# demox-labs/aleo

Hardware: AMD Instinct MI355X
Metric: MSM G1 scalar-muls/sec (2^20 bases per GPU, BLS12-377, bit-exact) (higher is better)
Workload: dtype u32

## Files before the change

aleo_amd/csrc/bases.hip:

```cpp
#include "entry.h"
#include "g2.h"
#include <cstdlib>
#include <cstring>

namespace aleo_mi355x {

struct RowFormat { size_t packed, strided; int32_t (*unpack)(Ctx* c, const void* d_rows, void* d_xy, void* d_flags, size_t n, hipStream_t s); };
static int32_t unpack_g2_200(Ctx* c, const void* d_rows, void* d_xy, void* d_flags, size_t n, hipStream_t s) {
  return g2_unpack200(d_rows, d_xy, d_flags, (uint32_t*)((char*)d_flags + ((n + 3) & ~(size_t)3)), n, s);
}
static constexpr RowFormat G1_ROWS = {96, 104, unpack_affine104}, G2_ROWS = {192, 200, unpack_g2_200};

static int32_t stage_rows(Ctx* c, const RowFormat& f, const void* rows, size_t stride, size_t n, void* d_xy, void* d_raw, void* d_flags, uint32_t* n_inf) {
  *n_inf = 0;
  if (!n) return ALEO_MI355X_OK;
  if (stride == f.packed) { HIPCHK(hipMemcpyAsync(d_xy, rows, n * f.packed, hipMemcpyHostToDevice, c->stream)); return ALEO_MI355X_OK; }
  HIPCHK(hipMemcpyAsync(d_raw, rows, n * f.strided, hipMemcpyHostToDevice, c->stream));
  if (int32_t rc = f.unpack(c, d_raw, d_xy, d_flags, n, c->stream)) return rc;
  HIPCHK(hipMemcpyAsync(n_inf, (char*)d_flags + ((n + 3) & ~(size_t)3), 4, hipMemcpyDeviceToHost, c->stream));
  HIPCHK(hipStreamSynchronize(c->stream));
  return ALEO_MI355X_OK;
}
static int32_t stage_rows_owned(Ctx* c, const RowFormat& f, const void* rows, size_t stride, size_t n, void** d_xy, uint8_t** d_inf) {
  DevTmp raw, flags; uint32_t n_inf = 0; int32_t rc;
// ... 19 lines not shown
}
static int32_t cold_bases(Ctx* c, const void* bases, size_t stride, size_t n, PinnedBases* pb) {
  *pb = PinnedBases(); pb->n = n; int32_t rc; const uint8_t* d_inf = nullptr;
  if ((rc = stage_rows_cold(c, G1_ROWS, bases, stride, n, &d_inf)) || (rc = c->cold_xy28.reserve((n ? n : 1) * ROW28))) return rc;
  pb->d_xy = c->cold_xy.p; pb->d_inf = (uint8_t*)d_inf;
  if ((rc = rows_to28_into(pb->d_xy, c->cold_xy28.p, n, c->stream))) return rc;
  pb->d_xy28 = c->cold_xy28.p;
  return ALEO_MI355X_OK;
}
template <class T> static uint64_t register_set(Device* d, std::map<uint64_t, std::shared_ptr<T>>& table, std::shared_ptr<T> o) {
  std::lock_guard<std::mutex> lk(d->mu);
  uint64_t h = d->next_handle++; table[h] = std::move(o); return h;
}
int32_t find_bases(Device* d, uint64_t handle, std::shared_ptr<PinnedOwner>* keep, PinnedBases* snap) {
  std::lock_guard<std::mutex> lk(d->mu);
  if (int32_t rc = handle_get(d->bases, handle, "unknown bases handle", keep)) return rc;
  *snap = (*keep)->pb; return ALEO_MI355X_OK;
}
template <class T> static int32_t unpin(Device* d, std::map<uint64_t, std::shared_ptr<T>>& table, uint64_t handle, const char* unknown) {
  std::shared_ptr<T> dead;
  std::lock_guard<std::mutex> lk(d->mu);
  return handle_get(table, handle, unknown, &dead, true);
}
static int32_t precompute_once(Ctx* c, const std::shared_ptr<PinnedOwner>& o) {
  Device* d = c->dev; PinnedBases work;
  {
    std::lock_guard<std::mutex> lk(d->mu);
    if (o->pb.tabled || o->building) return ALEO_MI355X_OK;
    o->building = true; work = o->pb;
  }
  int32_t rc = msm_precompute(c, &work);
  std::lock_guard<std::mutex> lk(d->mu);
  o->building = false;
  if (rc == ALEO_MI355X_OK) { for (int i = 0; i < 3; ++i) o->pb.tab[i] = work.tab[i]; o->pb.tabled = true; }
  return rc;
}

static bool looks_sparse(const void* scalars, size_t n) {
  if (n < 4096) return false;
  const uint64_t* s = (const uint64_t*)scalars; size_t small = 0; const size_t step = n / 257;
  for (size_t i = 0; i < 257; ++i) { const uint64_t* v = s + 4 * (i * step); small += (v[1] | v[2] | v[3]) == 0 && v[0] < (1ull << 32); }
  return small >= 129;
}
int32_t msm_host_scalars(Ctx* c, void* out, const PinnedBases& pb, const void* scalars, size_t n, bool mont) {
  const bool skewed = !mont && looks_sparse(scalars, n);
  const bool sparse = skewed && pb.range.d && pb.range_off == 0 && n <= pb.range.cover;
  if (!n) return msm_run1(c, (uint64_t*)out, pb, nullptr, 0, mont, c->stream, false);
  return msm_run1_split(c, (uint64_t*)out, pb, nullptr, n, mont, c->stream, sparse, scalars, !skewed);
}

static uint64_t hash96(const uint8_t* p) {
  uint64_t h = 1469598103934665603ull;
  for (int i = 0; i < 96; ++i) { h ^= p[i]; h *= 1099511628211ull; }
  return h;
}
static constexpr size_t SRS_SAMPLES = 256, SRS_CACHE_ENTRIES = 8, SRS_MIN_N = 1024;

static bool srs_cache_enabled() {
  const char* e = std::getenv("ALEO_MI355X_SRS_CACHE");
  return e && e[0] == '1';
}
static SrsCacheEntry* srs_lookup(Device* d, const void* bases, size_t stride, size_t n) {
  for (auto& e : d->srs_cache) {
    if (e.host_ptr != bases || e.stride != stride || e.n < n) continue;
    bool ok = true; size_t checked = 0;
    for (auto& sm : e.samples) {
      if (sm.first >= n) continue;
// ... 94 lines not shown
  });
}

int32_t aleo_mi355x_bases_generate(const void* base104, uint64_t first, size_t n, uint64_t* handle) {
  return guarded([&] {
    if (!base104 || !handle) return ALEO_MI355X_ERR_BAD_ARG;
    return pin_new(handle, [&](Ctx* c, std::shared_ptr<PinnedOwner>* o) { *o = std::make_shared<PinnedOwner>(); return generate_multiples(c, base104, first, n, &(*o)->pb); });
  });
}

int32_t aleo_mi355x_bases_from_scalars(const void* base104, const void* scalars, size_t n, uint64_t* handle) {
  return guarded([&] {
    if (!base104 || !handle || !scalars) return ALEO_MI355X_ERR_BAD_ARG;
    return pin_new(handle, [&](Ctx* c, std::shared_ptr<PinnedOwner>* o) { *o = std::make_shared<PinnedOwner>(); return generate_from_scalars(c, base104, scalars, n, &(*o)->pb); });
  });
}

int32_t aleo_mi355x_bases_precompute(uint64_t handle) {
  return guarded([&] {
    Slot sl; if (sl.rc) return sl.rc;
    FoundBases fb(sl.d, handle); if (fb.rc) return fb.rc;
    return precompute_once(sl.c, fb.keep);
  });
}

int32_t aleo_mi355x_bases_precompute_range(uint64_t handle, size_t offset, size_t n, int32_t window_bits) {
  return guarded([&] {
    Slot sl; if (sl.rc) return sl.rc;
    std::shared_ptr<PinnedOwner> keep; PinnedBases work; { int32_t rcb = find_bases(sl.d, handle, &keep, &work); if (rcb) return rcb; }
    { std::lock_guard<std::mutex> g(sl.d->mu); if (keep->building) return bad_arg("bases_precompute_range: a table build is in flight"); keep->building = true; work = keep->pb; }
    int32_t rc = msm_precompute_range(sl.c, &work, offset, n, window_bits);
    std::lock_guard<std::mutex> g(sl.d->mu);
    keep->building = false;
    if (rc == ALEO_MI355X_OK) { keep->pb.range = work.range; keep->pb.range_off = work.range_off; }
    return rc;
  });
}

int32_t aleo_mi355x_bases_info(uint64_t handle, uint64_t* out, int32_t cap) {
  return guarded([&] {
    if (!out || cap <= 0) return 0;
    Device* d = nullptr; if (get_device(&d)) return 0;
    std::shared_ptr<PinnedOwner> keep; PinnedBases pb; if (find_bases(d, handle, &keep, &pb)) return 0;
    uint64_t v[8] = {pb.n, pb.n * (96 + ROW28) + (pb.d_inf ? pb.n : 0), 0, 0, 0, 0, 0, 0};
    int k = 0;
    for (const auto& t : pb.tab) if (t.d) { const uint64_t W = (254 + t.c - 1) / t.c; v[2] += W * t.cover * ROW28; v[3 + k] = (uint64_t)t.c; ++k; }
    v[6] = (uint64_t)k;
    const int32_t m = cap < 8 ? cap : 8;
    for (int32_t i = 0; i < m; ++i) out[i] = v[i];
    return m;
  }, 0);
}

int32_t aleo_mi355x_bases_download(uint64_t handle, size_t offset, size_t n, void* out104) {
  return guarded([&] {
    if (!out104 && n) return ALEO_MI355X_ERR_BAD_ARG;
    Slot sl; if (sl.rc) return sl.rc;
    FoundBases fb(sl.d, handle); if (fb.rc) return fb.rc;
    if (offset + n > fb.pb.n) return bad_arg("bases_download: range");
    std::vector<uint8_t> xy(n * 96 + 1), inf(n + 1, 0);
    HIPCHK(hipMemcpy(xy.data(), (const char*)fb.pb.d_xy + offset * 96, n * 96, hipMemcpyDeviceToHost));
    if (fb.pb.d_inf) HIPCHK(hipMemcpy(inf.data(), fb.pb.d_inf + offset, n, hipMemcpyDeviceToHost));
    uint8_t* o = (uint8_t*)out104;
    for (size_t i = 0; i < n; ++i) { std::memcpy(o + i * 104, &xy[i * 96], 96); std::memset(o + i * 104 + 96, 0, 8); o[i * 104 + 96] = inf[i]; }
    return ALEO_MI355X_OK;
  });
}

int32_t aleo_mi355x_bases_unpin(uint64_t handle) {
  return guarded([&] { Slot sl; if (sl.rc) return sl.rc; return unpin(sl.d, sl.d->bases, handle, "unknown bases handle"); });
}

int32_t aleo_mi355x_bases_g2_pin(const void* bases, size_t base_stride, size_t n, uint64_t* handle) {
  return guarded([&] {
    if (!handle || (!bases && n) || (base_stride != 200 && base_stride != 192) || n >= (1ull << 31)) return bad_arg("bases_g2_pin: bad argument");
    Slot sl; if (sl.rc) return sl.rc;
    std::shared_ptr<PinnedG2> o;
    const int32_t rc = g2_upload(sl.c, bases, base_stride, n, &o);
    if (rc) return rc;
// ... 10 lines not shown
```

aleo_amd/csrc/ctx.h:

```cpp
#pragma once
#include <hip/hip_runtime.h>
#include <atomic>
#include <condition_variable>
#include <cstdint>
#include <cstdio>
#include <map>
#include <memory>
#include <functional>
#include <mutex>
#include <string>
#include <vector>
#include "../../include/aleo_mi355x.h"

namespace aleo_mi355x {

extern thread_local std::string g_last_error;

#define HIPCHK(expr)                                                                                   \
  do {                                                                                                 \
    hipError_t e__ = (expr);                                                                           \
    if (e__ != hipSuccess) {                                                                           \
      char buf__[512];                                                                                 \
      snprintf(buf__, sizeof buf__, "%s failed: %s (%s:%d)", #expr, hipGetErrorString(e__), __FILE__, __LINE__); \
      g_last_error = buf__;                                                                            \
      return (e__ == hipErrorOutOfMemory) ? ALEO_MI355X_ERR_OOM : ALEO_MI355X_ERR_HIP;                 \
    }                                                                                                  \
  } while (0)

struct DevBuf {
  void* p = nullptr; size_t cap = 0;
  int32_t reserve(size_t bytes) {
    if (bytes <= cap) return ALEO_MI355X_OK;
    if (p) { (void)hipFree(p); p = nullptr; cap = 0; }
    size_t want = bytes + bytes / 8;
    HIPCHK(hipMalloc(&p, want));
    cap = want; return ALEO_MI355X_OK;
  }
  template <class T> T* as() const { return (T*)p; }
};

struct Carve { size_t total = 0; size_t part(size_t bytes) { const size_t at = total; total += (bytes + 31) & ~(size_t)31; return at; } };

struct DevTmp {
  void* p = nullptr;
  DevTmp() = default; DevTmp(const DevTmp&) = delete; DevTmp& operator=(const DevTmp&) = delete;
  ~DevTmp() { if (p) (void)hipFree(p); }
  int32_t alloc(size_t bytes) { HIPCHK(hipMalloc(&p, bytes ? bytes : 1)); return ALEO_MI355X_OK; }
  void* release() { void* q = p; p = nullptr; return q; }
};

#ifndef ALEO_ROW28
#define ALEO_ROW28 128
#endif
static constexpr size_t ROW28 = ALEO_ROW28;
static_assert(ROW28 == 112 || ROW28 == 128, "row stride of the 28-bit tables");

struct PinnedBases {
  void* d_xy = nullptr;
  void* d_xy28 = nullptr;
  uint8_t* d_inf = nullptr;
  struct PreTable { void* d = nullptr; int c = 0; size_t cover = 0, min_n = 0; };
  PreTable tab[3];
  PreTable range; size_t range_off = 0;
  bool tabled = false;
  uint64_t shards = 0; size_t shard_min = 0;
  size_t shard_ntt_min = (size_t)1 << 24;
  size_t n = 0;
};

struct PinnedOwner {
  PinnedBases pb; bool building = false;
  ~PinnedOwner() { if (pb.d_xy) (void)hipFree(pb.d_xy); if (pb.d_xy28) (void)hipFree(pb.d_xy28); if (pb.d_inf) (void)hipFree(pb.d_inf); for (auto& t : pb.tab) if (t.d) (void)hipFree(t.d); if (pb.range.d) (void)hipFree(pb.range.d); }
};

struct PinnedG2 {
  void* d_xy = nullptr; uint8_t* d_inf = nullptr; void* d_rows28 = nullptr; size_t n = 0;
  ~PinnedG2() { if (d_xy) (void)hipFree(d_xy); if (d_inf) (void)hipFree(d_inf); if (d_rows28) (void)hipFree(d_rows28); }
};

struct SrsCacheEntry {
  const void* host_ptr = nullptr; size_t n = 0, stride = 0; uint64_t handle = 0, last_use = 0; uint32_t hits = 0;
  std::vector<std::pair<size_t, uint64_t>> samples;
};

struct MsmTiming { double total = 0, sort = 0, accum = 0, reduce = 0, host = 0, accum_kernel = 0; int accum_launches = 1; };

struct NttTables;

struct Device;

struct Ctx {
  Device* dev = nullptr;
  int device = -1;
  hipStream_t stream = nullptr;
  std::mutex mu;
  hipEvent_t ev[8] = {};
  uint32_t meta_seq = 0;
// ... 115 lines not shown
```

aleo_amd/csrc/g1_setup.hip:

```cpp
#include "ec.h"
#include "fp28.h"
#include "msm_common.h"

namespace aleo_mi355x {

static constexpr uint32_t GEN_K = 64;
__device__ __constant__ uint32_t FQ_P_MINUS_2[12] = {0xffffffffu, 0x8508bfffu, 0x30000000u, 0x170b5d44u, 0xba094800u, 0x1ef3622fu,
                                                     0x00f5138fu, 0x1a22d9f3u, 0x6ca1493bu, 0xc63b05c0u, 0x17c510eau, 0x01ae3a46u};
__device__ __noinline__ void fq_mul_ni(Fq* r, const Fq* a, const Fq* b) { *r = Fq::mul(*a, *b); }
__device__ __noinline__ void fq_inverse_ni(Fq* io) {
  Fq a = *io, acc = Fq::one();
  for (int bit = 376; bit >= 0; --bit) {
    fq_mul_ni(&acc, &acc, &acc);
    if ((FQ_P_MINUS_2[bit >> 5] >> (bit & 31)) & 1u) fq_mul_ni(&acc, &acc, &a);
  }
  *io = acc;
}

__global__ void __launch_bounds__(256) k_gen_xyzz(const char* __restrict__ g_affine, uint64_t first, uint32_t n, char* __restrict__ tmp) {
  uint32_t t = blockIdx.x * 256 + threadIdx.x;
  uint64_t i0 = (uint64_t)t * GEN_K; if (i0 >= n) return;
  AffinePt g = load_affine(g_affine);
  XYZZ G; G.X = g.x; G.Y = g.y; G.ZZ = Fq::one(); G.ZZZ = Fq::one();
  uint64_t k = first + i0;
  XYZZ acc = xyzz_infinity();
  for (int bit = 63 - __clzll(k); bit >= 0; --bit) {
    xyzz_double_ni(&acc);
    if ((k >> bit) & 1ull) xyzz_add_ni(&acc, &G);
  }
  for (uint32_t j = 0; j < GEN_K && i0 + j < n; ++j) {
    store_xyzz(tmp + (i0 + j) * 192, acc);
    xyzz_add_ni(&acc, &G);
  }
}
// ... 113 lines not shown
  (void)c;
  uint32_t* count = (uint32_t*)((char*)d_flags + ((n + 3) & ~(size_t)3));
  HIPCHK(hipMemsetAsync(count, 0, 4, s));
  const size_t want = (n + 255) / 256;
  hipLaunchKernelGGL(k_unpack104, dim3((uint32_t)(want < 16384 ? want : 16384)), dim3(256), 0, s, (const char*)d_rows104, (char*)d_xy96, (uint8_t*)d_flags, count, n);
  HIPCHK(hipGetLastError());
  return ALEO_MI355X_OK;
}

__global__ void __launch_bounds__(256) k_rows_to28(const char* __restrict__ src96, char* __restrict__ dst112, uint32_t n) {
  uint32_t i = blockIdx.x * 256 + threadIdx.x; if (i >= n) return;
  AffinePt p = load_affine(src96 + (size_t)i * 96);
  F28 x, y;
  if (p.x.is_zero_raw() && p.y.is_zero_raw()) { x = f28_const(Limbs14{}); y = x; }
  else { x = f28_from_fq(p.x); y = f28_from_fq(p.y); }
  store_affine28(dst112 + (size_t)i * ROW28, x, y);
}
int32_t rows_to28_into(const void* d_xy96, void* d_dst, size_t n, hipStream_t s) {
  if (n == 0) return ALEO_MI355X_OK;
  hipLaunchKernelGGL(k_rows_to28, dim3((uint32_t)((n + 255) / 256)), dim3(256), 0, s, (const char*)d_xy96, (char*)d_dst, (uint32_t)n);
  HIPCHK(hipGetLastError());
  return ALEO_MI355X_OK;
}
int32_t make_rows28(Ctx* c, PinnedBases* pb) {
  if (pb->d_xy28 || pb->n == 0) return ALEO_MI355X_OK;
  DevTmp rows; int32_t rc;
  if ((rc = rows.alloc(pb->n * ROW28))) return rc;
  if ((rc = rows_to28_into(pb->d_xy, rows.p, pb->n, c->stream))) return rc;
  HIPCHK(hipStreamSynchronize(c->stream));
  pb->d_xy28 = rows.release();
  return ALEO_MI355X_OK;
}

static int32_t build_table(Ctx* c, const PinnedBases* pb, int pre_c, size_t n, PinnedBases::PreTable* out, size_t off = 0) {
  const uint32_t W = (SCALAR_BITS + pre_c - 1) / pre_c;
  if (n * (size_t)W >= (1ull << 31)) { g_last_error = "bases_precompute: table index would exceed 31 bits"; return ALEO_MI355X_ERR_BAD_ARG; }
  DevTmp tab, cur, prefix, row; int32_t rc;
  if ((rc = tab.alloc(n * ROW28 * W))) return rc;
  if ((rc = cur.alloc(n * 192)) || (rc = prefix.alloc(n * 48)) || (rc = row.alloc(n * 96))) return rc;
  hipStream_t s = c->stream;
  const uint32_t g = (uint32_t)((n + 255) / 256), lanes = (uint32_t)((n + GEN_K - 1) / GEN_K), gl = (lanes + 255) / 256;
  const char* xy = (const char*)pb->d_xy + off * 96;
  if (pb->d_xy28) HIPCHK(hipMemcpyAsync(tab.p, (const char*)pb->d_xy28 + off * ROW28, n * ROW28, hipMemcpyDeviceToDevice, s));
  else hipLaunchKernelGGL(k_rows_to28, dim3(g), dim3(256), 0, s, xy, (char*)tab.p, (uint32_t)n);
  hipLaunchKernelGGL(k_pre_init, dim3(g), dim3(256), 0, s, xy, (uint32_t)n, (char*)cur.p);
  for (uint32_t w = 1; w < W; ++w) {
    hipLaunchKernelGGL(k_pre_double, dim3(g), dim3(256), 0, s, (char*)cur.p, (uint32_t)n, win_width(pre_c, (int)w - 1));
    hipLaunchKernelGGL(k_gen_normalize, dim3(gl), dim3(256), 0, s, (char*)cur.p, (uint32_t)n, (char*)prefix.p, (char*)row.p);
    hipLaunchKernelGGL(k_rows_to28, dim3(g), dim3(256), 0, s, (const char*)row.p, (char*)tab.p + (size_t)w * n * ROW28, (uint32_t)n);
  }
  HIPCHK(hipGetLastError());
  HIPCHK(hipStreamSynchronize(s));
  out->d = tab.release(); out->c = pre_c; out->cover = n;
  return ALEO_MI355X_OK;
}

int32_t msm_precompute(Ctx* c, PinnedBases* pb) {
  if (pb->tabled || pb->n == 0) return ALEO_MI355X_OK;
  const size_t N = pb->n; int32_t rc = ALEO_MI355X_OK; int k = 0;
  auto lim = [&](size_t cap) { return N < cap ? N : cap; };
  auto tier = [&](int cbits, size_t cover, size_t min_n) {
    if (rc) return;
    if ((rc = build_table(c, pb, cbits, cover, &pb->tab[k])) == ALEO_MI355X_OK) pb->tab[k++].min_n = min_n;
  };
  constexpr size_t TIER_SLACK = 64;
  const size_t cover16 = lim(((size_t)1 << 17) + TIER_SLACK), cover13 = lim(((size_t)1 << 15) + TIER_SLACK);
  if (N > cover16) tier(N >= (1u << 19) ? 20 : 17, N, cover16 + 1);
  if (N >= (1u << 15)) tier(16, cover16, (size_t)1 << 15);
  if (N >= (1u << 10)) tier(13, cover13, (size_t)1 << 10);
  if (rc) {
    for (auto& t : pb->tab) { if (t.d) (void)hipFree(t.d); t = PinnedBases::PreTable(); }
    return rc;
  }
  pb->tabled = true;
  return ALEO_MI355X_OK;
}

int32_t msm_precompute_range(Ctx* c, PinnedBases* pb, size_t off, size_t n, int window_bits) {
  if (pb->range.d) { g_last_error = "bases_precompute_range: this set already has a range table"; return ALEO_MI355X_ERR_BAD_ARG; }
  if (!n || off + n > pb->n || (window_bits != 13 && window_bits != 16)) { g_last_error = "bases_precompute_range: bad range or window (13 or 16 bits)"; return ALEO_MI355X_ERR_BAD_ARG; }
  int32_t rc = build_table(c, pb, window_bits, n, &pb->range, off);
  if (rc) return rc;
  pb->range.min_n = 0; pb->range_off = off;
  return ALEO_MI355X_OK;
}

}
```

aleo_amd/csrc/msm.hip:

```cpp
#include "msm_reduce.h"

namespace aleo_mi355x {

__device__ __forceinline__ XYZZ xyzz28_to_xyzz(const XYZZ28& a) {
  XYZZ r; r.X = f28_to_fq(a.X); r.Y = f28_to_fq(a.Y); r.ZZ = f28_to_fq(a.ZZ); r.ZZZ = f28_to_fq(a.ZZZ); return r;
}
__device__ __noinline__ void slice_slow_path28(const char* bases, const uint32_t* run, uint32_t j, uint32_t j1, const XYZZ28* acc28, XYZZ* acc_out, bool* inf_out) {
  XYZZ acc = xyzz28_to_xyzz(*acc28); bool inf = false;
  for (; j < j1; ++j) {
    uint32_t e = run[j];
    F28 x, y; load_affine28(bases + (size_t)(e & 0x7fffffffu) * ROW28, x, y);
    AffinePt p; p.x = Fq::reduce(f28_to_fq(x)); p.y = Fq::reduce(f28_to_fq(y));
    if (e >> 31) p.y = fq_neg_canonical(p.y);
    xyzz_madd(acc, inf, p.x, p.y);
  }
  *acc_out = acc; *inf_out = inf;
}

__device__ __forceinline__ const char* chain_sum(const FrontChain& ch, uint32_t g) {
  for (uint32_t i = 0; i < ch.n; ++i) if (ch.v[i].hist[g]) return ch.v[i].partial + (size_t)scan_at(ch.v[i].scan_local, ch.v[i].scan_blk, g).y * 224u;
  return nullptr;
}

template <bool OUT28, bool SEED = false>
__global__ void __launch_bounds__(256) k_accum28(const char* __restrict__ bases, const uint32_t* __restrict__ sorted, const uint32_t* __restrict__ hist,
                                                 const uint2* __restrict__ scan_local, const uint2* __restrict__ scan_blk, const uint32_t* __restrict__ total_pairs, uint32_t M,
                                                 const uint32_t* __restrict__ meta, const uint32_t* __restrict__ order, const uint32_t* __restrict__ task_g,
                                                 char* __restrict__ partial, FrontChain seed) {
  uint32_t t = blockIdx.x * 256 + threadIdx.x;
  if (t >= meta[0]) return;
  const uint32_t sid = order[t], g = task_g[sid];
  uint2 st = scan_at(scan_local, scan_blk, g);
  uint32_t cnt = hist[g], m = slices_of(cnt, pick_rule(total_pairs, M)), k = sid - st.y;
  uint32_t j0 = (uint32_t)(((uint64_t)k * cnt) / m), j1 = (uint32_t)(((uint64_t)(k + 1) * cnt) / m);
  const uint32_t* run = sorted + st.x;
  uint32_t e_next = run[j0];
  F28 xn, yn; load_affine28(bases + (size_t)(e_next & 0x7fffffffu) * ROW28, xn, yn);
  XYZZ28 acc; bool ok = true;
  uint32_t j = j0;
  bool seeded = false;
  if constexpr (SEED) {
    const char* sp = k == 0 ? chain_sum(seed, g) : nullptr;
    if (sp) {
      acc.ZZ = load_f28(sp + 112);
      if (!f28_is_zero_raw(acc.ZZ)) { acc.X = load_f28(sp); acc.Y = f28_mul(load_f28(sp + 56), f28_const(ONE28)); acc.ZZZ = load_f28(sp + 168); seeded = true; }
    }
  }
  if (!seeded) {
    uint32_t e = e_next; F28 x = xn, y = yn;
    if (j + 1 < j1) { e_next = run[j + 1]; load_affine28(bases + (size_t)(e_next & 0x7fffffffu) * ROW28, xn, yn); }
    if (e >> 31) y = f28_sub<2, 1>(f28_const(Limbs14{}), y);
    acc.X = x; acc.Y = y; acc.ZZ = f28_const(ONE28); acc.ZZZ = f28_const(ONE28);
    ++j;
  }
// ... 240 lines not shown
  ((uint4*)out)[t] = ((const uint4*)(V + (size_t)w * stride * PB28))[q];
}

int32_t msm_front_sort(Ctx* c, const PinnedBases& pb, const MsmJob& job, hipStream_t s, Front& f) {
  const uint32_t K = f.K = job.k;
  size_t n = 0, pts = 0; SegArgs segs{};
  if (K > MAX_SETS || job.nseg > MAX_SEGS) { g_last_error = "msm: too many sets / segments in one call"; return ALEO_MI355X_ERR_BAD_ARG; }
  for (uint32_t q = 0; q < job.nseg; ++q) {
    const MsmSeg& g = job.segs[q];
    if (g.len == 0) continue;
    if (g.out >= K || g.off + g.len >= (1ull << 31)) { g_last_error = "msm: segment out of range"; return ALEO_MI355X_ERR_BAD_ARG; }
    const uint32_t i = segs.nseg++;
    segs.ptr[i] = (const char*)g.d_ptr; segs.n[i] = (uint32_t)g.len; segs.off[i] = (uint32_t)g.off; segs.set[i] = (uint8_t)g.out;
    n = g.off + g.len > n ? g.off + g.len : n; pts += g.len;
  }
  if (n == 0) { f.empty = true; return ALEO_MI355X_OK; }
  if (job.tier_n > n && job.tier_n <= pb.n) n = job.tier_n;
  if (n > pb.n) { g_last_error = "msm: a segment reaches past the pinned bases"; return ALEO_MI355X_ERR_BAD_ARG; }
  const PinnedBases::PreTable* T = nullptr;
  const uint8_t* d_inf = pb.d_inf;
  bool ranged = job.sparse && pb.range.d != nullptr;
  for (uint32_t i = 0; ranged && i < segs.nseg; ++i) ranged = segs.off[i] >= pb.range_off && (size_t)segs.off[i] + segs.n[i] <= pb.range_off + pb.range.cover;
  if (ranged) {
    T = &pb.range; n = 0;
    for (uint32_t i = 0; i < segs.nseg; ++i) { segs.off[i] -= (uint32_t)pb.range_off; n = (size_t)segs.off[i] + segs.n[i] > n ? (size_t)segs.off[i] + segs.n[i] : n; }
    if (d_inf) d_inf += pb.range_off;
  } else T = msm_tier(pb, n);
  const bool pre = f.pre = T != nullptr;
  if (K > 1 && (!pre || K > (ranged ? msm_range_sets(pb) : msm_max_sets(pb, n)))) { g_last_error = "msm: internal: batch without a table tier (or too many sets)"; return ALEO_MI355X_ERR_BAD_ARG; }
  MsmPlan& P = f.P; P = make_plan(pre ? n : pts, pre ? T->c : 0);
  if (pre) { P.W = K; P.M = K * P.B; }
  if (!pre && !pb.d_xy28) { g_last_error = "msm: pinned set without 28-bit rows"; return ALEO_MI355X_ERR_HIP; }
  f.bases = (const char*)(pre ? T->d : pb.d_xy28);
  f.plain_tree = k_tree_pass<Pt32, 2>;
  const uint32_t cpw = f.cpw = P.B / P.S, nchunks = f.nchunks = cpw * P.W;
  uint32_t lgN = 0; while ((1u << lgN) < cpw) ++lgN;
  f.lgN = lgN;
  const bool masked = f.masked = pre && lgN >= 2 && (1u << lgN) == cpw;
  if (pre && !masked) { g_last_error = "msm: internal: table path without masked reduction"; return ALEO_MI355X_ERR_HIP; }
  int32_t rc;
  const uint32_t tseg = f.tseg = cpw / 4, fseg = f.fseg = lgN + 4, nseg = f.nseg = K * fseg, setw = f.setw = fseg * tseg;
  constexpr uint32_t SUM_TREE_MIN_C = 13;
  f.prog = masked && P.c >= SUM_TREE_MIN_C && cpw > FOLD;
  f.out_pts = f.prog ? 1 + lgN : fseg;
  f.vpoints = masked ? (size_t)K * setw + nchunks + (nseg + 1) + (size_t)nseg * (tseg / 2 + tseg / 4 + 2) + 3 * (size_t)nchunks + 64 : (size_t)nchunks + P.W;
  if ((rc = ensure_host_pinned(c, 64 + (size_t)(masked ? nseg : P.W) * 224 + ASIDE_MAX * 228))) return rc;
  SortPhase& sp = f.sp;
  if ((rc = msm_sort_phase(c, segs, pts, job.mont, d_inf, (uint32_t)(pre ? T->cover : pb.n), P, pre, s, &sp, f.lean))) return rc;
  const uint32_t M = sp.M;
  if ((rc = c->partial.reserve(sp.slices_max * (pre ? 224 : 192)))) return rc;
  if ((rc = c->vbuf.reserve(f.vpoints * 224))) return rc;
  return ALEO_MI355X_OK;
}

int32_t msm_front_accum(Ctx* c, hipStream_t s, Front& f, const FrontChain* seed, hipEvent_t after) {
  const SortPhase& sp = f.sp; const uint32_t M = sp.M; const char* bases = f.bases;
  char* partial = c->partial.as<char>();
  if (after) HIPCHK(hipStreamWaitEvent(s, after, 0));
  if (!f.lean) HIPCHK(hipEventRecord(c->ev[6], s));
  const bool seeded = f.pre && seed && seed->n;
  auto* const kern = seeded ? k_accum28<true, true> : f.pre ? k_accum28<true, false> : k_accum28<false, false>;
  hipLaunchKernelGGL(kern, dim3(sp.slice_blocks), dim3(256), 0, s, bases, sp.sorted, sp.hist, sp.scan_local, sp.scan_blk, sp.total_pairs, M, sp.meta, sp.order, sp.task_g, partial, seeded ? *seed : FrontChain{});
  if (!f.lean) HIPCHK(hipEventRecord(c->ev[5], s));
  HIPCHK(hipGetLastError());
  return ALEO_MI355X_OK;
}

int32_t msm_front_finish(Ctx* c, hipStream_t s, Front& f, bool allow_aside) {
  int32_t rc;
  const SortPhase& sp = f.sp; SliceMeta& sm = f.sm; const uint32_t M = sp.M; const bool pre = f.pre;
  uint32_t* heavy = sp.heavy; uint32_t* meta = sp.meta; uint2* scan_local = sp.scan_local; uint2* scan_blk = sp.scan_blk;
  char* partial = c->partial.as<char>();
  if ((rc = msm_wait_meta(c, sp, s, &sm))) return rc;
  const bool aside = f.aside = allow_aside && f.masked && sm.n_super >= 1 && sm.n_super <= ASIDE_MAX && !sm.super_overflow && sm.max_m >= 64;
  uint32_t* h_aside = (uint32_t*)((char*)c->h_pinned + 64 + (size_t)f.nseg * 224);
  if (aside) {
    if (f.lean) HIPCHK(hipEventRecord(c->ev[5], s));
    HIPCHK(hipStreamWaitEvent(c->side, c->ev[5], 0));
    for (uint32_t pass = 0, L = sm.max_m - 1; L > 1; ++pass, L = (L + 1) >> 1) {
      const uint64_t ops = (uint64_t)sm.n_super * (L >> 1);
      launch_grp(grp_lanes(ops), k_tree_pass<Pt28, 4>, k_tree_pass<Pt28, 2>, ops, c->side, partial, heavy, 0u, 0u, sp.super_list, sm.n_super, L >> 1, scan_local, scan_blk, M, meta, pass, 1u);
    }
    uint32_t* dst = nullptr;
    HIPCHK(hipHostGetDevicePointer((void**)&dst, h_aside, 0));
    hipLaunchKernelGGL(k_gather_super, dim3((sm.n_super * 57 + 255) / 256), dim3(256), 0, c->side, partial, sp.super_list, sm.n_super, scan_local, scan_blk, dst);
    HIPCHK(hipEventRecord(c->ev[4], c->side));
  }
  const bool rest_ok = pre && !sm.super_overflow && (aside || sm.n_super == 0) && sm.n_heavy && sm.max_common > 2 && sm.max_common <= 8;
  if (sm.NT) {
    for (uint32_t pass = 0, L = sm.max_m, Lcm = sm.max_common; L > 1; ++pass, L = (L + 1) >> 1, Lcm = (Lcm + 1) >> 1) {
      if (rest_ok && pass == 1) {
        hipLaunchKernelGGL(k_tree_rest<4>, dim3((uint32_t)((4ull * sm.n_heavy + 255) / 256)), dim3(256), 0, s, partial, heavy, sm.n_heavy, scan_local, scan_blk, M, meta);
        break;
      }
      const uint32_t Lc = sm.super_overflow ? L : Lcm;
// ... 218 lines not shown
```

aleo_amd/csrc/msm_chain.h:

```cpp
#pragma once
#include "msm_common.h"
#include <chrono>

namespace aleo_mi355x {
#pragma GCC visibility push(hidden)
struct FrontView { const char* partial; const uint32_t* hist; const uint2* scan_local; const uint2* scan_blk; };
struct FrontChain { FrontView v[3]; uint32_t n = 0; };
struct Front {
  MsmPlan P{}; SortPhase sp; SliceMeta sm;
  uint32_t K = 0, cpw = 0, nchunks = 0, lgN = 0, tseg = 0, fseg = 0, nseg = 0, setw = 0; size_t vpoints = 0;
  uint32_t out_pts = 0;
  bool pre = false, masked = false, prog = false, aside = false, empty = false, lean = false; const char* bases = nullptr;
  void (*plain_tree)(char*, const uint32_t*, uint32_t, uint32_t, const uint32_t*, uint32_t, uint32_t, const uint2*, const uint2*, uint32_t, const uint32_t*, uint32_t, uint32_t) = nullptr;
};
struct StreamDrainGuard {
  std::vector<hipStream_t> streams; bool armed = true;
  ~StreamDrainGuard() { if (!armed) return; const std::string keep = g_last_error; for (hipStream_t st : streams) if (st) (void)hipStreamSynchronize(st); g_last_error = keep; }
  void add(hipStream_t st) { streams.push_back(st); }
  void dismiss() { armed = false; }
};
int32_t msm_front_sort(Ctx* c, const PinnedBases& pb, const MsmJob& job, hipStream_t s, Front& f);
int32_t msm_front_accum(Ctx* c, hipStream_t s, Front& f, const FrontChain* seed, hipEvent_t after);
int32_t msm_front_finish(Ctx* c, hipStream_t s, Front& f, bool allow_aside);
int32_t msm_reduce_queue(Ctx* c, Front& f, hipStream_t s, const FrontChain& older);
enum class TailWait { stream, event };
int32_t msm_collect(Ctx* c, uint64_t* out_jac18, Front& f, hipStream_t s, bool fire_tail, TailWait wait);
int32_t msm_back(Ctx* c, uint64_t* out_jac18, Front& f, hipStream_t s, bool fire_tail, const FrontChain& older);
int32_t phase_times(Ctx* c, const Front& f, std::chrono::steady_clock::time_point t_host0);
#pragma GCC visibility pop
}
```

aleo_amd/msm.py:

```python
from __future__ import annotations
import ctypes
import numpy as np
from ._lib import lib, check


def _p(a): return a.ctypes.data_as(ctypes.c_void_p)


class PinnedBases:

    def __init__(self, bases: np.ndarray = None, _handle: int = 0, _n: int = 0):
        if bases is None:
            self.handle, self.n = _handle, _n
            return
        bases = np.ascontiguousarray(bases, dtype=np.uint8)
        assert bases.ndim == 2 and bases.shape[1] in (96, 104)
        self.n = bases.shape[0]
        h = ctypes.c_uint64(0)
        check(lib().aleo_mi355x_bases_pin(_p(bases), bases.shape[1], self.n, ctypes.byref(h)), 'bases_pin')
        self.handle = h.value

    @classmethod
    def generate_multiples(cls, base_affine104: np.ndarray, first_multiple: int, n: int) -> 'PinnedBases':
        b = np.ascontiguousarray(base_affine104, dtype=np.uint8).reshape(104)
        h = ctypes.c_uint64(0)
        check(lib().aleo_mi355x_bases_generate(_p(b), first_multiple, n, ctypes.byref(h)), 'bases_generate')
        return cls(None, h.value, n)

    @classmethod
    def from_scalars(cls, base_affine104: np.ndarray, scalars: np.ndarray) -> 'PinnedBases':
        b = np.ascontiguousarray(base_affine104, dtype=np.uint8).reshape(104)
        sc = np.ascontiguousarray(scalars, dtype=np.uint64).reshape(-1, 4)
        h = ctypes.c_uint64(0)
        check(lib().aleo_mi355x_bases_from_scalars(_p(b), _p(sc), sc.shape[0], ctypes.byref(h)), 'bases_from_scalars')
        return cls(None, h.value, sc.shape[0])

    def precompute(self) -> 'PinnedBases':
        check(lib().aleo_mi355x_bases_precompute(self.handle), 'bases_precompute')
        return self

    def precompute_range(self, offset: int, n: int, window_bits: int = 13) -> 'PinnedBases':
        check(lib().aleo_mi355x_bases_precompute_range(self.handle, offset, n, window_bits), 'bases_precompute_range')
        return self

    def info(self) -> dict:
        buf = (ctypes.c_uint64 * 8)()
        k = lib().aleo_mi355x_bases_info(self.handle, buf, 8)
        if k < 7: raise ValueError('unknown bases handle')
        return {'points': int(buf[0]), 'row_bytes': int(buf[1]), 'table_bytes': int(buf[2]), 'tier_window_bits': [int(buf[3 + i]) for i in range(int(buf[6]))]}

    def attach_shards(self, sharded: 'ShardedBases' = None, min_points: int = 0, transforms_from: int = None) -> 'PinnedBases':
        check(lib().aleo_mi355x_bases_attach_shards(self.handle, sharded.handle if sharded is not None else 0, int(min_points)), 'bases_attach_shards')
        if sharded is not None and transforms_from is not None:
            check(lib().aleo_mi355x_bases_shard_transforms(self.handle, int(transforms_from)), 'bases_shard_transforms')
        return self

    def download(self, offset: int = 0, n: int = None) -> np.ndarray:
        n = self.n - offset if n is None else n
        out = np.zeros((n, 104), dtype=np.uint8)
        check(lib().aleo_mi355x_bases_download(self.handle, offset, n, _p(out)), 'bases_download')
        return out

    def close(self):
        if self.handle:
            lib().aleo_mi355x_bases_unpin(self.handle); self.handle = 0

    def __enter__(self): return self
    def __exit__(self, *a): self.close()
    def __del__(self):
        try: self.close()
        except Exception: pass


class ShardedBases:

    def __init__(self, bases: np.ndarray = None, devices=1, precompute: bool = False, _handle: int = 0, _n: int = 0):
        if bases is None:
            self.handle, self.n = _handle, _n
            return
        bases = np.ascontiguousarray(bases, dtype=np.uint8)
        assert bases.ndim == 2 and bases.shape[1] in (96, 104)
        self.n = bases.shape[0]
# ... 133 lines not shown
```

Before: 369.1 million.

## Store precomputed tables in twisted Edwards form and accumulate with extended coordinates

After a subgroup check on the pinned bases, precomputed window tables are built in twisted Edwards (y-x, y+x, 2dxy) rows. Bucket accumulation then runs a new Edwards mixed-add kernel, converting to and from XYZZ at the boundaries. The aim is to replace XYZZ mixed additions with the cheaper, branch-free unified Edwards addition. In exchange, table rows grow to 192 bytes (more memory traffic), there are extra conversion costs, and precompute gains a subgroup scan.

```diff
diff --git a/aleo_amd/csrc/bases.hip b/aleo_amd/csrc/bases.hip
--- a/aleo_amd/csrc/bases.hip
+++ b/aleo_amd/csrc/bases.hip
@@ -75,7 +75,7 @@
   int32_t rc = msm_precompute(c, &work);
   std::lock_guard<std::mutex> lk(d->mu);
   o->building = false;
-  if (rc == ALEO_MI355X_OK) { for (int i = 0; i < 3; ++i) o->pb.tab[i] = work.tab[i]; o->pb.tabled = true; }
+  if (rc == ALEO_MI355X_OK) { for (int i = 0; i < 3; ++i) o->pb.tab[i] = work.tab[i]; o->pb.tabled = true; o->pb.subgroup = work.subgroup; }
   return rc;
 }
 
@@ -236,7 +236,7 @@
     int32_t rc = msm_precompute_range(sl.c, &work, offset, n, window_bits);
     std::lock_guard<std::mutex> g(sl.d->mu);
     keep->building = false;
-    if (rc == ALEO_MI355X_OK) { keep->pb.range = work.range; keep->pb.range_off = work.range_off; }
+    if (rc == ALEO_MI355X_OK) { keep->pb.range = work.range; keep->pb.range_off = work.range_off; keep->pb.subgroup = work.subgroup; }
     return rc;
   });
 }
@@ -248,7 +248,7 @@
     std::shared_ptr<PinnedOwner> keep; PinnedBases pb; if (find_bases(d, handle, &keep, &pb)) return 0;
     uint64_t v[8] = {pb.n, pb.n * (96 + ROW28) + (pb.d_inf ? pb.n : 0), 0, 0, 0, 0, 0, 0};
     int k = 0;
-    for (const auto& t : pb.tab) if (t.d) { const uint64_t W = (254 + t.c - 1) / t.c; v[2] += W * t.cover * ROW28; v[3 + k] = (uint64_t)t.c; ++k; }
+    for (const auto& t : pb.tab) if (t.d) { const uint64_t W = (254 + t.c - 1) / t.c; v[2] += W * t.cover * t.row_bytes(); v[3 + k] = (uint64_t)t.c; v[7] = (uint64_t)t.form; ++k; }
     v[6] = (uint64_t)k;
     const int32_t m = cap < 8 ? cap : 8;
     for (int32_t i = 0; i < m; ++i) out[i] = v[i];
diff --git a/aleo_amd/csrc/ctx.h b/aleo_amd/csrc/ctx.h
--- a/aleo_amd/csrc/ctx.h
+++ b/aleo_amd/csrc/ctx.h
@@ -54,15 +54,25 @@
 #endif
 static constexpr size_t ROW28 = ALEO_ROW28;
 static_assert(ROW28 == 112 || ROW28 == 128, "row stride of the 28-bit tables");
+#ifndef ALEO_TE_ROW
+#define ALEO_TE_ROW 192
+#endif
+static constexpr size_t TE_ROW = ALEO_TE_ROW;
+static_assert(TE_ROW >= 168 && TE_ROW % 64 == 0, "row stride of the twisted Edwards tables");
+enum TableForm : int { TABLE_WEIERSTRASS = 0, TABLE_EDWARDS = 1 };
 
 struct PinnedBases {
   void* d_xy = nullptr;
   void* d_xy28 = nullptr;
   uint8_t* d_inf = nullptr;
-  struct PreTable { void* d = nullptr; int c = 0; size_t cover = 0, min_n = 0; };
+  struct PreTable {
+    void* d = nullptr; int c = 0; size_t cover = 0, min_n = 0; int form = TABLE_WEIERSTRASS;
+    size_t row_bytes() const { return form == TABLE_EDWARDS ? TE_ROW : ROW28; }
+  };
   PreTable tab[3];
   PreTable range; size_t range_off = 0;
   bool tabled = false;
+  int subgroup = -1;
   uint64_t shards = 0; size_t shard_min = 0;
   size_t shard_ntt_min = (size_t)1 << 24;
   size_t n = 0;
diff --git a/aleo_amd/csrc/g1_setup.hip b/aleo_amd/csrc/g1_setup.hip
--- a/aleo_amd/csrc/g1_setup.hip
+++ b/aleo_amd/csrc/g1_setup.hip
@@ -1,5 +1,6 @@
 #include "ec.h"
 #include "fp28.h"
+#include "te28.h"
 #include "msm_common.h"
 
 namespace aleo_mi355x {
@@ -179,32 +180,110 @@
   return ALEO_MI355X_OK;
 }
 
+__device__ __constant__ uint32_t FR_MODULUS_WORDS[8] = {0x00000001u, 0x0a118000u, 0xd0000001u, 0x59aa76feu, 0x5c37b001u, 0x60b44d1eu, 0x9a2ca556u, 0x12ab655eu};
+__global__ void __launch_bounds__(256) k_subgroup_check(const char* __restrict__ xy, const uint8_t* __restrict__ inf, uint32_t n, uint32_t* __restrict__ n_bad) {
+  uint32_t i = blockIdx.x * 256 + threadIdx.x; if (i >= n) return;
+  const AffinePt p = load_affine(xy + (size_t)i * 96);
+  if ((inf && inf[i]) || (p.x.is_zero_raw() && p.y.is_zero_raw())) return;
+  Fq xx, x3, yy; fq_mul_ni(&xx, &p.x, &p.x); fq_mul_ni(&x3, &xx, &p.x); fq_mul_ni(&yy, &p.y, &p.y);
+  bool bad = !Fq::sub<4>(Fq::add(x3, Fq::one()), yy).is_zero_mod();
+  XYZZ P; P.X = p.x; P.Y = p.y; P.ZZ = Fq::one(); P.ZZZ = Fq::one();
+  XYZZ acc = xyzz_infinity();
+#pragma unroll 1
+  for (int w = 7; w >= 0; --w) {
+    const uint32_t word = FR_MODULUS_WORDS[w];
+#pragma unroll 1
+    for (int b = 31; b >= 0; --b) {
+      xyzz_double_ni(&acc);
+      if ((word >> b) & 1u) xyzz_add_ni(&acc, &P);
+    }
+  }
+  bad = bad || !(xyzz_is_inf(acc) || acc.ZZ.is_zero_mod());
+  if (bad) atomicAdd(n_bad, 1u);
+}
+static int32_t subgroup_gate(Ctx* c, PinnedBases* pb) {
+  if (pb->subgroup >= 0) return ALEO_MI355X_OK;
+  DevTmp cnt; int32_t rc;
+  if ((rc = cnt.alloc(4))) return rc;
+  HIPCHK(hipMemsetAsync(cnt.p, 0, 4, c->stream));
+  hipLaunchKernelGGL(k_subgroup_check, dim3((uint32_t)((pb->n + 255) / 256)), dim3(256), 0, c->stream, (const char*)pb->d_xy, (const uint8_t*)pb->d_inf, (uint32_t)pb->n, (uint32_t*)cnt.p);
+  HIPCHK(hipGetLastError());
+  uint32_t n_bad = 0;
+  HIPCHK(hipMemcpyAsync(&n_bad, cnt.p, 4, hipMemcpyDeviceToHost, c->stream));
+  HIPCHK(hipStreamSynchronize(c->stream));
+  pb->subgroup = n_bad ? 0 : 1;
+  return ALEO_MI355X_OK;
+}
+
+__device__ __forceinline__ void te_uv(const AffinePt& p, const Fq& S, Fq& u, Fq& v, Fq& up1) {
+  u = Fq::mul(S, Fq::add(p.x, Fq::one())); v = Fq::mul(S, p.y); up1 = Fq::add(u, Fq::one());
+}
+__global__ void __launch_bounds__(256) k_rows_to_te(const char* __restrict__ src96, char* __restrict__ dst, uint32_t n, char* __restrict__ prefix) {
+  uint32_t t = blockIdx.x * 256 + threadIdx.x;
+  uint64_t i0 = (uint64_t)t * GEN_K; if (i0 >= n) return;
+  uint32_t cnt = (uint32_t)((n - i0) < GEN_K ? (n - i0) : GEN_K);
+  const Fq S = f28_to_fq(f28_const(TE28_S)), K = f28_to_fq(f28_const(TE28_KAPPA)), D2 = Fq::dbl(f28_to_fq(f28_const(TE28_D)));
+  Fq prod = Fq::one();
+  for (uint32_t j = 0; j < cnt; ++j) {
+    store_fp<Fq>(prefix + (i0 + j) * 48, prod);
+    const AffinePt p = load_affine(src96 + (i0 + j) * 96);
+    Fq u, v, up1; te_uv(p, S, u, v, up1);
+    Fq den; fq_mul_ni(&den, &v, &up1);
+    if ((p.x.is_zero_raw() && p.y.is_zero_raw()) || den.is_zero_mod_lt2p()) den = Fq::one();
+    fq_mul_ni(&prod, &prod, &den);
+  }
+  fq_inverse_ni(&prod);
+  for (uint32_t jj = cnt; jj-- > 0;) {
+    const AffinePt p = load_affine(src96 + (i0 + jj) * 96);
+    char* out = dst + (i0 + jj) * TE_ROW;
+    Fq u, v, up1; te_uv(p, S, u, v, up1);
+    Fq den; fq_mul_ni(&den, &v, &up1);
+    if ((p.x.is_zero_raw() && p.y.is_zero_raw()) || den.is_zero_mod_lt2p()) {
+      const F28 z = f28_const(Limbs14{}); store_te28_row(out, z, z, z);
+      continue;
+    }
+    const Fq pre = load_fp<Fq>(prefix + (i0 + jj) * 48);
+    Fq inv; fq_mul_ni(&inv, &prod, &pre);
+    fq_mul_ni(&prod, &prod, &den);
+    Fq a, b, xe, ye, xy;
+    fq_mul_ni(&a, &u, &up1); fq_mul_ni(&a, &a, &inv); fq_mul_ni(&xe, &K, &a);
+    b = Fq::sub<1>(u, Fq::one()); fq_mul_ni(&b, &b, &v); fq_mul_ni(&ye, &b, &inv);
+    fq_mul_ni(&xy, &xe, &ye); fq_mul_ni(&xy, &xy, &D2);
+    store_te28_row(out, f28_from_fq(Fq::sub<2>(ye, xe)), f28_from_fq(Fq::add(ye, xe)), f28_from_fq(xy));
+  }
+}
+
 static int32_t build_table(Ctx* c, const PinnedBases* pb, int pre_c, size_t n, PinnedBases::PreTable* out, size_t off = 0) {
   const uint32_t W = (SCALAR_BITS + pre_c - 1) / pre_c;
   if (n * (size_t)W >= (1ull << 31)) { g_last_error = "bases_precompute: table index would exceed 31 bits"; return ALEO_MI355X_ERR_BAD_ARG; }
+  PinnedBases::PreTable T; T.form = pb->subgroup == 1 ? TABLE_EDWARDS : TABLE_WEIERSTRASS;
+  const bool te = T.form == TABLE_EDWARDS; const size_t RB = T.row_bytes();
   DevTmp tab, cur, prefix, row; int32_t rc;
-  if ((rc = tab.alloc(n * ROW28 * W))) return rc;
+  if ((rc = tab.alloc(n * RB * W))) return rc;
   if ((rc = cur.alloc(n * 192)) || (rc = prefix.alloc(n * 48)) || (rc = row.alloc(n * 96))) return rc;
   hipStream_t s = c->stream;
   const uint32_t g = (uint32_t)((n + 255) / 256), lanes = (uint32_t)((n + GEN_K - 1) / GEN_K), gl = (lanes + 255) / 256;
   const char* xy = (const char*)pb->d_xy + off * 96;
-  if (pb->d_xy28) HIPCHK(hipMemcpyAsync(tab.p, (const char*)pb->d_xy28 + off * ROW28, n * ROW28, hipMemcpyDeviceToDevice, s));
+  if (te) hipLaunchKernelGGL(k_rows_to_te, dim3(gl), dim3(256), 0, s, xy, (char*)tab.p, (uint32_t)n, (char*)prefix.p);
+  else if (pb->d_xy28) HIPCHK(hipMemcpyAsync(tab.p, (const char*)pb->d_xy28 + off * ROW28, n * ROW28, hipMemcpyDeviceToDevice, s));
   else hipLaunchKernelGGL(k_rows_to28, dim3(g), dim3(256), 0, s, xy, (char*)tab.p, (uint32_t)n);
   hipLaunchKernelGGL(k_pre_init, dim3(g), dim3(256), 0, s, xy, (uint32_t)n, (char*)cur.p);
   for (uint32_t w = 1; w < W; ++w) {
     hipLaunchKernelGGL(k_pre_double, dim3(g), dim3(256), 0, s, (char*)cur.p, (uint32_t)n, win_width(pre_c, (int)w - 1));
     hipLaunchKernelGGL(k_gen_normalize, dim3(gl), dim3(256), 0, s, (char*)cur.p, (uint32_t)n, (char*)prefix.p, (char*)row.p);
-    hipLaunchKernelGGL(k_rows_to28, dim3(g), dim3(256), 0, s, (const char*)row.p, (char*)tab.p + (size_t)w * n * ROW28, (uint32_t)n);
+    if (te) hipLaunchKernelGGL(k_rows_to_te, dim3(gl), dim3(256), 0, s, (const char*)row.p, (char*)tab.p + (size_t)w * n * RB, (uint32_t)n, (char*)prefix.p);
+    else hipLaunchKernelGGL(k_rows_to28, dim3(g), dim3(256), 0, s, (const char*)row.p, (char*)tab.p + (size_t)w * n * RB, (uint32_t)n);
   }
   HIPCHK(hipGetLastError());
   HIPCHK(hipStreamSynchronize(s));
-  out->d = tab.release(); out->c = pre_c; out->cover = n;
+  T.d = tab.release(); T.c = pre_c; T.cover = n; *out = T;
   return ALEO_MI355X_OK;
 }
 
 int32_t msm_precompute(Ctx* c, PinnedBases* pb) {
   if (pb->tabled || pb->n == 0) return ALEO_MI355X_OK;
   const size_t N = pb->n; int32_t rc = ALEO_MI355X_OK; int k = 0;
+  if (N >= (1u << 10) && (rc = subgroup_gate(c, pb))) return rc;
   auto lim = [&](size_t cap) { return N < cap ? N : cap; };
   auto tier = [&](int cbits, size_t cover, size_t min_n) {
     if (rc) return;
@@ -226,8 +305,8 @@
 int32_t msm_precompute_range(Ctx* c, PinnedBases* pb, size_t off, size_t n, int window_bits) {
   if (pb->range.d) { g_last_error = "bases_precompute_range: this set already has a range table"; return ALEO_MI355X_ERR_BAD_ARG; }
   if (!n || off + n > pb->n || (window_bits != 13 && window_bits != 16)) { g_last_error = "bases_precompute_range: bad range or window (13 or 16 bits)"; return ALEO_MI355X_ERR_BAD_ARG; }
-  int32_t rc = build_table(c, pb, window_bits, n, &pb->range, off);
-  if (rc) return rc;
+  int32_t rc = subgroup_gate(c, pb);
+  if (rc || (rc = build_table(c, pb, window_bits, n, &pb->range, off))) return rc;
   pb->range.min_n = 0; pb->range_off = off;
   return ALEO_MI355X_OK;
 }
diff --git a/aleo_amd/csrc/msm.hip b/aleo_amd/csrc/msm.hip
--- a/aleo_amd/csrc/msm.hip
+++ b/aleo_amd/csrc/msm.hip
@@ -15,11 +15,6 @@
     xyzz_madd(acc, inf, p.x, p.y);
   }
   *acc_out = acc; *inf_out = inf;
-}
-
-__device__ __forceinline__ const char* chain_sum(const FrontChain& ch, uint32_t g) {
-  for (uint32_t i = 0; i < ch.n; ++i) if (ch.v[i].hist[g]) return ch.v[i].partial + (size_t)scan_at(ch.v[i].scan_local, ch.v[i].scan_blk, g).y * 224u;
-  return nullptr;
 }
 
 template <bool OUT28, bool SEED = false>
@@ -326,6 +321,7 @@
   if (pre) { P.W = K; P.M = K * P.B; }
   if (!pre && !pb.d_xy28) { g_last_error = "msm: pinned set without 28-bit rows"; return ALEO_MI355X_ERR_HIP; }
   f.bases = (const char*)(pre ? T->d : pb.d_xy28);
+  f.te = pre && T->form == TABLE_EDWARDS;
   f.plain_tree = k_tree_pass<Pt32, 2>;
   const uint32_t cpw = f.cpw = P.B / P.S, nchunks = f.nchunks = cpw * P.W;
   uint32_t lgN = 0; while ((1u << lgN) < cpw) ++lgN;
@@ -353,8 +349,11 @@
   if (after) HIPCHK(hipStreamWaitEvent(s, after, 0));
   if (!f.lean) HIPCHK(hipEventRecord(c->ev[6], s));
   const bool seeded = f.pre && seed && seed->n;
-  auto* const kern = seeded ? k_accum28<true, true> : f.pre ? k_accum28<true, false> : k_accum28<false, false>;
-  hipLaunchKernelGGL(kern, dim3(sp.slice_blocks), dim3(256), 0, s, bases, sp.sorted, sp.hist, sp.scan_local, sp.scan_blk, sp.total_pairs, M, sp.meta, sp.order, sp.task_g, partial, seeded ? *seed : FrontChain{});
+  if (f.te) launch_accum_te28(f, partial, seeded ? seed : nullptr, s);
+  else {
+    auto* const kern = seeded ? k_accum28<true, true> : f.pre ? k_accum28<true, false> : k_accum28<false, false>;
+    hipLaunchKernelGGL(kern, dim3(sp.slice_blocks), dim3(256), 0, s, bases, sp.sorted, sp.hist, sp.scan_local, sp.scan_blk, sp.total_pairs, M, sp.meta, sp.order, sp.task_g, partial, seeded ? *seed : FrontChain{});
+  }
   if (!f.lean) HIPCHK(hipEventRecord(c->ev[5], s));
   HIPCHK(hipGetLastError());
   return ALEO_MI355X_OK;
diff --git a/aleo_amd/csrc/msm_chain.h b/aleo_amd/csrc/msm_chain.h
--- a/aleo_amd/csrc/msm_chain.h
+++ b/aleo_amd/csrc/msm_chain.h
@@ -6,11 +6,15 @@
 #pragma GCC visibility push(hidden)
 struct FrontView { const char* partial; const uint32_t* hist; const uint2* scan_local; const uint2* scan_blk; };
 struct FrontChain { FrontView v[3]; uint32_t n = 0; };
+__device__ __forceinline__ const char* chain_sum(const FrontChain& ch, uint32_t g) {
+  for (uint32_t i = 0; i < ch.n; ++i) if (ch.v[i].hist[g]) return ch.v[i].partial + (size_t)scan_at(ch.v[i].scan_local, ch.v[i].scan_blk, g).y * 224u;
+  return nullptr;
+}
 struct Front {
   MsmPlan P{}; SortPhase sp; SliceMeta sm;
   uint32_t K = 0, cpw = 0, nchunks = 0, lgN = 0, tseg = 0, fseg = 0, nseg = 0, setw = 0; size_t vpoints = 0;
   uint32_t out_pts = 0;
-  bool pre = false, masked = false, prog = false, aside = false, empty = false, lean = false; const char* bases = nullptr;
+  bool pre = false, te = false, masked = false, prog = false, aside = false, empty = false, lean = false; const char* bases = nullptr;
   void (*plain_tree)(char*, const uint32_t*, uint32_t, uint32_t, const uint32_t*, uint32_t, uint32_t, const uint2*, const uint2*, uint32_t, const uint32_t*, uint32_t, uint32_t) = nullptr;
 };
 struct StreamDrainGuard {
@@ -21,6 +25,7 @@
 };
 int32_t msm_front_sort(Ctx* c, const PinnedBases& pb, const MsmJob& job, hipStream_t s, Front& f);
 int32_t msm_front_accum(Ctx* c, hipStream_t s, Front& f, const FrontChain* seed, hipEvent_t after);
+void launch_accum_te28(const Front& f, char* partial, const FrontChain* seed, hipStream_t s);
 int32_t msm_front_finish(Ctx* c, hipStream_t s, Front& f, bool allow_aside);
 int32_t msm_reduce_queue(Ctx* c, Front& f, hipStream_t s, const FrontChain& older);
 enum class TailWait { stream, event };
diff --git a/aleo_amd/csrc/msm_te.hip b/aleo_amd/csrc/msm_te.hip
--- /dev/null
+++ b/aleo_amd/csrc/msm_te.hip
@@ -0,0 +1,52 @@
+#include "msm_chain.h"
+#include "te28.h"
+
+namespace aleo_mi355x {
+
+template <bool SEED>
+__global__ void __launch_bounds__(256) k_accum_te28(const char* __restrict__ rows, const uint32_t* __restrict__ sorted, const uint32_t* __restrict__ hist,
+                                                    const uint2* __restrict__ scan_local, const uint2* __restrict__ scan_blk, const uint32_t* __restrict__ total_pairs, uint32_t M,
+                                                    const uint32_t* __restrict__ meta, const uint32_t* __restrict__ order, const uint32_t* __restrict__ task_g,
+                                                    char* __restrict__ partial, FrontChain seed) {
+  uint32_t t = blockIdx.x * 256 + threadIdx.x;
+  if (t >= meta[0]) return;
+  const uint32_t sid = order[t], g = task_g[sid];
+  uint2 st = scan_at(scan_local, scan_blk, g);
+  uint32_t cnt = hist[g], m = slices_of(cnt, pick_rule(total_pairs, M)), k = sid - st.y;
+  uint32_t j0 = (uint32_t)(((uint64_t)k * cnt) / m), j1 = (uint32_t)(((uint64_t)(k + 1) * cnt) / m);
+  const uint32_t* run = sorted + st.x;
+  uint32_t e_next = run[j0];
+  F28 n0, n1, n2; load_te28_row(rows + (size_t)(e_next & 0x7fffffffu) * TE_ROW, n0, n1, n2);
+  TE28 acc;
+  uint32_t j = j0;
+  bool seeded = false;
+  if constexpr (SEED) {
+    const char* sp = k == 0 ? chain_sum(seed, g) : nullptr;
+    if (sp) {
+      XYZZ28 p; p.ZZ = load_f28(sp + 112);
+      if (!f28_is_zero_raw(p.ZZ)) { p.X = load_f28(sp); p.Y = load_f28(sp + 56); p.ZZZ = load_f28(sp + 168); acc = te28_from_xyzz28(p); seeded = true; }
+    }
+  }
+  if (!seeded) {
+    uint32_t e = e_next; F28 r0 = n0, r1 = n1, r2 = n2;
+    if (j + 1 < j1) { e_next = run[j + 1]; load_te28_row(rows + (size_t)(e_next & 0x7fffffffu) * TE_ROW, n0, n1, n2); }
+    te28_row_sign(e >> 31, r0, r1, r2);
+    acc = te28_first(r0, r1, r2);
+    ++j;
+  }
+  for (; j < j1; ++j) {
+    uint32_t e = e_next; F28 r0 = n0, r1 = n1, r2 = n2;
+    if (j + 1 < j1) { e_next = run[j + 1]; load_te28_row(rows + (size_t)(e_next & 0x7fffffffu) * TE_ROW, n0, n1, n2); }
+    te28_row_sign(e >> 31, r0, r1, r2);
+    te28_madd(acc, r0, r1, r2);
+  }
+  store_xyzz28(partial + (size_t)sid * 224, te28_to_xyzz28(acc));
+}
+
+void launch_accum_te28(const Front& f, char* partial, const FrontChain* seed, hipStream_t s) {
+  const SortPhase& sp = f.sp;
+  auto* const kern = seed ? k_accum_te28<true> : k_accum_te28<false>;
+  hipLaunchKernelGGL(kern, dim3(sp.slice_blocks), dim3(256), 0, s, f.bases, sp.sorted, sp.hist, sp.scan_local, sp.scan_blk, sp.total_pairs, sp.M, sp.meta, sp.order, sp.task_g, partial, seed ? *seed : FrontChain{});
+}
+
+}
diff --git a/aleo_amd/csrc/te28.h b/aleo_amd/csrc/te28.h
--- /dev/null
+++ b/aleo_amd/csrc/te28.h
@@ -0,0 +1,101 @@
+#pragma once
+#ifndef ALEO_F28_PROVIDED
+#include "fp28.h"
+
+namespace aleo_mi355x {
+
+__device__ __forceinline__ void load_te28_row(const void* p, F28& r0, F28& r1, F28& r2) {
+  const uint4* s = (const uint4*)p; uint32_t w[44];
+#pragma unroll
+  for (int i = 0; i < 10; ++i) { uint4 t = s[i]; w[4 * i] = t.x; w[4 * i + 1] = t.y; w[4 * i + 2] = t.z; w[4 * i + 3] = t.w; }
+  const uint2 t = ((const uint2*)p)[20]; w[40] = t.x; w[41] = t.y;
+#pragma unroll
+  for (int i = 0; i < 14; ++i) { r0.v[i] = w[i]; r1.v[i] = w[14 + i]; r2.v[i] = w[28 + i]; }
+}
+__device__ __forceinline__ void store_te28_row(void* p, const F28& r0, const F28& r1, const F28& r2) {
+  uint32_t w[44];
+#pragma unroll
+  for (int i = 0; i < 14; ++i) { w[i] = r0.v[i]; w[14 + i] = r1.v[i]; w[28 + i] = r2.v[i]; }
+  uint4* d = (uint4*)p;
+#pragma unroll
+  for (int i = 0; i < 10; ++i) d[i] = make_uint4(w[4 * i], w[4 * i + 1], w[4 * i + 2], w[4 * i + 3]);
+  ((uint2*)p)[20] = make_uint2(w[40], w[41]);
+}
+
+}
+#endif
+
+namespace aleo_mi355x {
+
+static constexpr Limbs14 TE28_S = {{0x01a0a113u, 0x0b0dad83u, 0x0c8df2c0u, 0x0c9ee451u, 0x01935a6eu, 0x06425e1bu, 0x0acf94dfu, 0x09d801ddu, 0x014590dbu, 0x0ad64a0cu, 0x02a17c35u, 0x06b6b819u, 0x00112a8cu, 0x00000fa6u}};
+static constexpr Limbs14 TE28_INV_S = {{0x04e1e338u, 0x009d0889u, 0x05a9d7bdu, 0x000869f5u, 0x0cb9f841u, 0x0fcb79bcu, 0x014fcb3bu, 0x0d78b460u, 0x09add89fu, 0x066e4a72u, 0x0cdeb434u, 0x03157be7u, 0x05ed67e0u, 0x0000140eu}};
+static constexpr Limbs14 TE28_KAPPA = {{0x0605e344u, 0x09db8eadu, 0x0c7a99c9u, 0x053cf352u, 0x06254f3bu, 0x007ad145u, 0x0769ac1au, 0x0eb261abu, 0x0a5ececdu, 0x0625c845u, 0x0568b26eu, 0x037d10bau, 0x084097bau, 0x00000867u}};
+static constexpr Limbs14 TE28_D = {{0x03836291u, 0x0f402225u, 0x047d3f76u, 0x04a2fad5u, 0x0aeb7224u, 0x08dcfc19u, 0x093b36e6u, 0x08f1a17fu, 0x06683e85u, 0x0e5de8a7u, 0x097017b0u, 0x0ef7a07cu, 0x0d19b13eu, 0x0000197bu}};
+static constexpr Limbs14 TE28_INV_D = {{0x0c7448d7u, 0x0d9fdddau, 0x072e84acu, 0x07593d2au, 0x051c3a60u, 0x0c66f1aeu, 0x09769153u, 0x0d87e5d4u, 0x05ca9538u, 0x07670b3cu, 0x049cf899u, 0x0ca3cb94u, 0x0b5300dbu, 0x00001a5eu}};
+static constexpr Limbs14 TE28_TWO = {{0x0ffecf58u, 0x041fffffu, 0x0f61ae4eu, 0x0d2407ffu, 0x049361c9u, 0x0c2e468au, 0x02abaee3u, 0x057f1355u, 0x06506764u, 0x031c22d7u, 0x0fb8b92fu, 0x01a87d26u, 0x05c66296u, 0x00000768u}};
+
+struct TE28 { F28 X, Y, Z, T; };
+
+__device__ __forceinline__ void te28_row_sign(bool neg, F28& r0, F28& r1, F28& r2) {
+  const F28 a = r0, n2 = f28_sub<2, 1>(f28_const(Limbs14{}), r2);
+  r0 = f28_sel(neg, a, r1); r1 = f28_sel(neg, r1, a); r2 = f28_sel(neg, r2, n2);
+}
+
+__device__ __forceinline__ TE28 te28_first(const F28& r0, const F28& r1, const F28& r2) {
+  TE28 a;
+  a.X = f28_normalise(f28_sub<2, 1>(r1, r0));
+  a.Y = f28_normalise(f28_add(r1, r0));
+  a.Z = f28_const(TE28_TWO);
+  a.T = f28_mul(r2, f28_const(TE28_INV_D));
+  return a;
+}
+
+__device__ __forceinline__ void te28_madd(TE28& acc, const F28& r0, const F28& r1, const F28& r2) {
+  const F28 A = f28_mul(f28_sub<4, 1>(acc.Y, acc.X), r0);
+  const F28 B = f28_mul(f28_add(acc.Y, acc.X), r1);
+  const F28 C = f28_mul(acc.T, r2);
+  const F28 D = f28_add(acc.Z, acc.Z);
+  const F28 E = f28_sub<4, 1>(B, A);
+  const F28 F = f28_sub<4, 1>(D, C);
+  const F28 G = f28_add(D, C);
+  const F28 H = f28_add(B, A);
+  acc.X = f28_mul(E, F);
+  acc.Y = f28_mul(G, H);
+  acc.Z = f28_mul(F, G);
+  acc.T = f28_mul(E, H);
+}
+
+__device__ __forceinline__ XYZZ28 te28_to_xyzz28(const TE28& acc) {
+  const F28 a = f28_sub<4, 1>(acc.Z, acc.Y);
+  const F28 b = f28_add(acc.Z, acc.Y);
+  const F28 D = f28_mul(a, acc.X);
+  const bool inf = f28_is_zero_mod_lt2q(D);
+  const F28 ZZ = f28_sqr(D);
+  const F28 ZZZ = f28_mul(D, ZZ);
+  const F28 isb = f28_mul(b, f28_const(TE28_INV_S));
+  const F28 DX = f28_mul(D, acc.X);
+  const F28 Xw = f28_mul(f28_sub<8, 3>(isb, a), DX);
+  const F28 k = f28_mul(isb, f28_const(TE28_KAPPA));
+  const F28 Yw = f28_mul(k, f28_mul(acc.Z, ZZ));
+  const F28 zero = f28_const(Limbs14{});
+  XYZZ28 r;
+  r.X = f28_sel(inf, Xw, zero); r.Y = f28_sel(inf, Yw, zero); r.ZZ = f28_sel(inf, ZZ, zero); r.ZZZ = f28_sel(inf, ZZZ, zero);
+  return r;
+}
+
+__device__ __forceinline__ TE28 te28_from_xyzz28(const XYZZ28& p) {
+  const F28 m = f28_add(p.X, p.ZZ);
+  const F28 nx = f28_mul(f28_mul(m, f28_const(TE28_KAPPA)), p.ZZZ);
+  const F28 dx = f28_mul(p.Y, p.ZZ);
+  const F28 sm = f28_mul(m, f28_const(TE28_S));
+  const F28 ny = f28_sub<4, 1>(sm, p.ZZ);
+  const F28 dy = f28_add(sm, p.ZZ);
+  TE28 a;
+  a.X = f28_mul(nx, dy);
+  a.Y = f28_mul(ny, dx);
+  a.Z = f28_mul(dx, dy);
+  a.T = f28_mul(nx, ny);
+  return a;
+}
+
+}
diff --git a/aleo_amd/msm.py b/aleo_amd/msm.py
--- a/aleo_amd/msm.py
+++ b/aleo_amd/msm.py
@@ -47,7 +47,8 @@
         buf = (ctypes.c_uint64 * 8)()
         k = lib().aleo_mi355x_bases_info(self.handle, buf, 8)
         if k < 7: raise ValueError('unknown bases handle')
-        return {'points': int(buf[0]), 'row_bytes': int(buf[1]), 'table_bytes': int(buf[2]), 'tier_window_bits': [int(buf[3 + i]) for i in range(int(buf[6]))]}
+        return {'points': int(buf[0]), 'row_bytes': int(buf[1]), 'table_bytes': int(buf[2]), 'tier_window_bits': [int(buf[3 + i]) for i in range(int(buf[6]))],
+                'table_form': (('weierstrass', 'edwards')[int(buf[7])] if k >= 8 and int(buf[6]) else None)}
 
     def attach_shards(self, sharded: 'ShardedBases' = None, min_points: int = 0, transforms_from: int = None) -> 'PinnedBases':
         check(lib().aleo_mi355x_bases_attach_shards(self.handle, sharded.handle if sharded is not None else 0, int(min_points)), 'bases_attach_shards')
```

Result: faster. 380.3 million (median of 6 runs) (+3.1%).
